# caojiezhang/CiaoSR

Hardware: AMD Instinct MI355X
Metric: HR Mpix/s (RDN-CiaoSR x4, LocalImplicitSR forward_test) (higher is better)
Workload: dtype f32; 1 GPU; C3: RDN-CiaoSR (c64b16) x4, LR 1356x2040 -> 5424x8160 (DIV2K-shaped 2K LR), tiled inference: 117 tiles of 192x192 (overlap 32), random-init weights, fp32; scale=4, tiles=117, parallelism=tile-shard x1

## Files before the change

ciaosr_amd/_lib.py:

```python
import ctypes as C
import os

_HERE = os.path.dirname(os.path.abspath(__file__))
LIB_PATH = os.environ.get('CIAOSR_HIP_LIB') or os.path.join(_HERE, 'csrc', 'libciaosr_hip.so')
MAX_LAYERS = 8

ACT_NONE, ACT_RELU, ACT_PRELU, ACT_GELU, ACT_SIN, ACT_COS = 0, 1, 2, 3, 4, 5


class CiaoSRHipError(RuntimeError):
    pass


class MlpT(C.Structure):
    _fields_ = [('n_layers', C.c_int), ('act', C.c_int), ('in_dim', C.c_int), ('width', C.c_int * MAX_LAYERS),
                ('weight', C.c_void_p * MAX_LAYERS), ('ld', C.c_int * MAX_LAYERS),
                ('bias', C.c_void_p * MAX_LAYERS), ('frag', C.c_void_p * MAX_LAYERS),
                ('frag16', C.c_void_p * MAX_LAYERS), ('frag16_lo', C.c_void_p * MAX_LAYERS)]


class HeadWeightsT(C.Structure):
    _fields_ = [('channels', C.c_int), ('nonlocal_channels', C.c_int), ('nonlocal_max_scale', C.c_int), ('local_size', C.c_int),
                ('no_unfold', C.c_int),
                ('softmax_scale', C.c_float), ('q', MlpT), ('k', MlpT), ('v', MlpT), ('k_out_wino', C.c_void_p), ('k_out_wino4', C.c_void_p),
# ... 6 lines not shown


class CsAttnWeightsT(C.Structure):
    _fields_ = [('channels', C.c_int), ('scale', C.c_int),
                ('w_match1', C.c_void_p), ('b_match1', C.c_void_p), ('slope_match1', C.c_float),
                ('w_match2', C.c_void_p), ('b_match2', C.c_void_p), ('slope_match2', C.c_float),
                ('w_assembly', C.c_void_p), ('b_assembly', C.c_void_p), ('slope_assembly', C.c_float),
                ('w_down', C.c_void_p), ('b_down', C.c_void_p), ('w_down_masked', C.c_void_p),
                ('escape_nan', C.c_float), ('softmax_scale', C.c_float)]


class OptionsT(C.Structure):
    _fields_ = [('head_route', C.c_int), ('csa_composed_min', C.c_int), ('dense_min_tiles', C.c_int),
                ('scatter_small_max', C.c_int), ('kv_rows', C.c_int), ('decode_rows', C.c_int), ('bf16_single', C.c_int),
                ('dense_direct', C.c_int), ('csa_scores_gemm', C.c_int), ('csa_attn_tile128', C.c_int), ('query_grid_w', C.c_int), ('f16_pairs', C.c_int),
                ('csa_attn_v16', C.c_int), ('edsr_resident', C.c_int), ('swin_h16', C.c_int), ('csa_block_mb', C.c_int)]


HEAD_STAGED, HEAD_NO_LOGIT_TABLE, HEAD_TABLE_GEMM, HEAD_WIDE_WG, HEAD_TABLE_WINO2, HEAD_NO_CHAIN, HEAD_NO_DECODE_CHAIN = 1, 2, 4, 8, 16, 32, 64


class ConvT(C.Structure):
    _fields_ = [('weight', C.c_void_p), ('bias', C.c_void_p), ('cin', C.c_int), ('cout', C.c_int), ('ksize', C.c_int),
                ('frag16', C.c_void_p), ('frag16_lo', C.c_void_p), ('frag', C.c_void_p), ('frag_wino', C.c_void_p),
                ('frag_wino4', C.c_void_p)]


class RdnWeightsT(C.Structure):
    _fields_ = [('mid_channels', C.c_int), ('growth', C.c_int), ('num_blocks', C.c_int), ('num_layers', C.c_int),
                ('sfe1', ConvT), ('sfe2', ConvT), ('gff0', ConvT), ('gff1', ConvT),
                ('dense', C.POINTER(ConvT)), ('lff', C.POINTER(ConvT)),
# ... 29 lines not shown
    'ciaosr_sizeof': (_S, [C.c_char_p]),
    'ciaosr_prof_enable': (_I, [_I]),
    'ciaosr_prof_filter': (_I, [C.c_char_p]),
    'ciaosr_prof_reset': (_I, []),
    'ciaosr_prof_collect': (_I, []),
    'ciaosr_prof_get': (_I, [C.c_char_p, C.POINTER(C.c_double), C.POINTER(C.c_long)]),
    'ciaosr_prof_names': (_I, [C.c_char_p, _I]),
    'ciaosr_nchw_to_hwc_f32': (_I, [_P, _P, _I, _I, _I, _I, _P]),
    'ciaosr_hwc_to_nchw_f32': (_I, [_P, _I, _P, _I, _I, _I, _P]),
    'ciaosr_gemm_f32': (_I, [_P, _I, _P, _I, _I, _P, _I, _P, _I, _I, _I, _F, _I, _F, _P]),
    'ciaosr_patch_rows_f32': (_I, [_P, _I, _I, _I, _I, _I, _I, _I, _I, _I, _P, _I, _I, _F, _P]),
    'ciaosr_cs_attn_workspace_bytes': (_S, [_I, _I, _I]),
    'ciaosr_cs_attn_workspace_bytes_scale': (_S, [_I, _I, _I, _I]),
    'ciaosr_cs_attn_workspace_bytes_opt': (_S, [_I, _I, _I, _I, _O]),
    'ciaosr_cs_attn_block_rows': (_I, [_I, _I, _I, _I, _I, _O]),
    'ciaosr_cs_attn_f32': (_I, [_P, _I, _I, _I, C.POINTER(CsAttnWeightsT), _P, _I, _O, _P, _S, _P]),
    'ciaosr_cs_attn_bf16': (_I, [_P, _I, _I, _I, C.POINTER(CsAttnWeightsT), _P, _I, _O, _P, _S, _P]),
    'ciaosr_make_coord_cell_f32': (_I, [_P, _P, _I, _I, _P]),
    'ciaosr_make_coord_cell_window_f32': (_I, [_P, _P, _I, _I, _I, _I, _I, _I, C.POINTER(_I), _P]),
    'ciaosr_fragment_floats': (_S, [_I, _I]),
    'ciaosr_head_decode_rows': (_I, [_I, _I]),
    'ciaosr_pack_fragments_f32': (_I, [_P, _I, _I, _I, _P, _P]),
    'ciaosr_cs_attn_f16': (_I, [_P, _I, _I, _I, C.POINTER(CsAttnWeightsT), _P, _I, _O, _P, _S, _P]),
    'ciaosr_fragment_bf16_bytes': (_S, [_I, _I]),
    'ciaosr_fragment_f16_bytes': (_S, [_I, _I]),
    'ciaosr_pack_fragments_f16': (_I, [_P, _I, _I, _I, _P, _P]),
    'ciaosr_pack_fragments_bf16': (_I, [_P, _I, _I, _I, _P, _P]),
    'ciaosr_pack_fragments_bf16_lo': (_I, [_P, _I, _I, _I, _P, _P]),
    'ciaosr_pack_fragments_f16_lo': (_I, [_P, _I, _I, _I, _P, _P]),
    'ciaosr_pack_fragments_bf16_pair': (_I, [_P, _I, _I, _I, _P, _P, _P]),
# ... 161 lines not shown
```

ciaosr_amd/csrc/common.h:

```cpp
#pragma once
#include <hip/hip_runtime.h>
#include <atomic>
#include <cstdint>
#include <cstdio>
#include <mutex>

#include "../../include/ciaosr_hip.h"

namespace ciaosr {

constexpr int kWave = 64;

static inline int ceil_div(long a, long b) { return (int)((a + b - 1) / b); }

static inline bool aligned16(const void* p) { return (reinterpret_cast<uintptr_t>(p) & 15u) == 0; }

struct ProfScope {
    int slot;
    hipStream_t stream;
    hipEvent_t ev0, ev1;
    ProfScope(const char* name, hipStream_t s);
    ~ProfScope();
};

// ... 19 lines not shown

__device__ __forceinline__ void wave_lds_sync() {
    __builtin_amdgcn_fence(__ATOMIC_RELEASE, "wavefront");
    __builtin_amdgcn_wave_barrier();
    __builtin_amdgcn_fence(__ATOMIC_ACQUIRE, "wavefront");
}

int launch_status(const char* what);

static inline bool options_ok(const ciaosr_options_t* o) {
    if (!o) return true;
    return o->query_grid_w >= 0 && (o->csa_attn_tile128 == 0 || o->csa_attn_tile128 == 1) && (o->head_route & ~127) == 0 && (o->kv_rows == 0 || o->kv_rows == 32 || o->kv_rows == 64) &&
           (o->decode_rows == 0 || o->decode_rows == 32 || o->decode_rows == 64) && (o->bf16_single == 0 || o->bf16_single == 1) &&
           (o->dense_direct >= 0 && o->dense_direct <= 2) && (o->csa_scores_gemm == 0 || o->csa_scores_gemm == 1) &&
           o->f16_pairs >= 0 && o->f16_pairs <= 3 && (o->csa_attn_v16 == 0 || o->csa_attn_v16 == 1) && o->csa_block_mb >= 0 &&
           (o->swin_h16 == 0 || o->swin_h16 == 1) && (o->edsr_resident == 0 || o->edsr_resident == 1);
}

}

#define CIAOSR_BIG_LDS(kernel, bytes)                                                              \
    do {                                                                                           \
        static ::ciaosr::LdsAttrOnce once_;                                                        \
        if (!::ciaosr::allow_big_lds(once_, kernel, bytes)) return CIAOSR_ERR_LAUNCH;              \
    } while (0)

#define CIAOSR_CHECK_ARG(cond)                                                         \
    do {                                                                               \
        if (!(cond)) {                                                                 \
            std::fprintf(stderr, "[ciaosr_hip] bad argument: %s (%s:%d)\n", #cond,     \
                         __FILE__, __LINE__);                                          \
// ... 4 lines not shown
```

ciaosr_amd/csrc/csattn.hip:

```cpp
#include "ops.h"

namespace ciaosr {

struct CsaPlan {
    int H, W, C, sc, Hp, Wp, HWp, Hl, Wl, L, Lld, Lld8, Ch;
    int band_rows, up, down, s_rows;
    size_t n_V, n_S, n_Y;
    bool banded() const { return band_rows < Hp; }
};

static CsaPlan csa_plan(int H, int W, int C, int sc) {
    CsaPlan p;
    p.H = H; p.W = W; p.C = C; p.sc = sc; p.Ch = (int)round_up(C / 2, 4);
    p.Hp = (int)round_up((size_t)H, sc); p.Wp = (int)round_up((size_t)W, sc);
    p.HWp = p.Hp * p.Wp; p.Hl = p.Hp / sc; p.Wl = p.Wp / sc; p.L = p.Hl * p.Wl;
    p.Lld = (int)round_up(p.L, 4); p.Lld8 = (int)round_up(p.L, 8);
    p.band_rows = p.s_rows = p.Hp; p.up = p.down = 0;
    p.n_V = (size_t)p.L * 9 * sc * sc * C; p.n_S = (size_t)p.HWp * p.Lld; p.n_Y = (size_t)sc * sc * p.HWp * C;
    return p;
}

static bool csa_composed(const CsaPlan& p, const ciaosr_options_t* opt) {
    const int composed_min = opt && opt->csa_composed_min ? opt->csa_composed_min : 4096;
    return p.sc == 2 && composed_min > 0 && p.HWp >= composed_min;
// ... 63 lines not shown
    b.Er = p.banded() ? take((size_t)(p.Wp + p.Hp) * p.Lld) : nullptr;
    return b;
}
static size_t csa_carve_bytes(const CsaPlan& p, bool p16) {
    size_t n = 0;
    csa_carve(p, p16, [&](size_t floats) { n += floats; return (float*)nullptr; });
    return n * sizeof(float) + 24 * 256;
}

enum CsaScores { kScoresBox, kScoresGemm, kScores16 };
enum CsaTail { kTailUncomposed, kTail16C, kTailFour, kTail16 };
struct CsaRoute {
    CsaScores scores; CsaTail tail;
    bool tile128;
    bool fused_softmax;
};

static CsaRoute csa_route(const CsaPlan& p, Prec prec, const ciaosr_options_t* opt, const ciaosr_csattn_weights_t* w) {
    CsaRoute r = {kScoresGemm, kTailUncomposed, opt && opt->csa_attn_tile128, false};
    if (prec == kF32 && !(opt && opt->csa_scores_gemm) && csa_scores_box_ok(p.Ch, p.Ch, p.Ch)) r.scores = kScoresBox;
    if (!(csa_composed(p, opt) && w->w_down_masked)) return r;
    if (prec != kF32 && (9 * p.Ch) % 8 == 0 && (p.Lld & 3) == 0 && qk16_fits(p) && vpt_fits(p)) {
        r.scores = kScores16; r.tail = kTail16;
        r.fused_softmax = softmax16_fits(p, h16_ops(prec)) && w->softmax_scale > 0.f;
    } else if (csa_wants_four(p, prec, opt, p.s_rows)) {
        r.tail = kTailFour;
    } else {
        r.tail = kTail16C;
    }
    return r;
}
static bool csa_attn_big(const CsaPlan& p, const CsaRoute& r, int M) {
    return !r.tile128 && gemm_big_softmax_f32_ok(p.Lld, 25 * p.C, M, 16 * p.C, p.L, true) &&
           ((size_t)(M - 1) * p.Lld + p.L) * sizeof(float) < 0xFFFFFF00ull;
}

// ... 54 lines not shown
    int patch_down(const float* src, int Hs, int Ws, int stride, int pad, int OH, int OW, float* dst) const {
        return patch_rows(src, C, Hs, Ws, C, 3, stride, pad, OH, OW, dst, 9 * C, 0, 0.f, s, "csa_patch_down");
    }
    int partial_down() const {
        CSA_RUN(patch_down(E, Hp, Wp, 2, 3, Hl + 3, Wl + 3, PE));
        return gemm_f32(PE, 9 * C, w->w_down_masked, 9 * C, false, Pc, 9 * C, nullptr, (Hl + 3) * (Wl + 3), 9 * C, 9 * C, 1.f, CIAOSR_ACT_NONE, 0.f, s,
                        "csa_down_partial");
    }

    int keep_edge_logits(const CsaBand& b) const {
        if (!banded()) return CIAOSR_OK;
        if (b.first()) CSA_RUN(copy_rows(S, Lld, Wp, Lld, edge_rows(), Lld, s, "csa_edge_rows"));
        return copy_rows(S + (size_t)(b.y0 - b.ya) * Wp * Lld, (long)Wp * Lld, b.y1 - b.y0, Lld, edge_rows() + (size_t)(Wp + b.y0) * Lld, Lld, s,
                         "csa_edge_rows");
    }
    int edges(const float* Vc, int ld, int col0, const float* probs) const {
        auto edge = [&](int pix0, int pix_stride, int col, float* dst, int rows, int n) -> int {
            const float* B = Vc + col0 + col;
            if (probs)
                return gemm_f32_splitk(probs + (size_t)pix0 * Lld, Lld, B, ld, true, dst, n, nullptr, rows, n, L, 1.f, CIAOSR_ACT_NONE, 0.f, splitk(),
                                       n_Y, s, "csa_attn_v_edge");
            const float* A = !banded() ? S : edge_rows() + (size_t)pix0 * Lld;
            return gemm_f32_softmax_a(A, banded() ? Lld : pix_stride * Lld, stats(), pix_stride, B, ld, true, dst, n, rows, n, L, splitk(), n_Y, s,
                                      "csa_attn_v_edge");
        };
        CSA_RUN(edge(0, 1, 0, otop(), Wp, 4 * C));
        CSA_RUN(edge(Wp, Wp, 4 * C, oleft(), Hp, 4 * C));
        return edge(0, 1, 8 * C, otl(), 1, C);
    }
    int finish_16c(const float* probs) const {
        CSA_RUN(edges(Vp, 25 * C, 16 * C, probs));
        return csa_gather_out(O, otop(), oleft(), otl(), w->b_down, H, W, Hp, Wp, C, out, ld_out, 16L * C, 4L * C, 4L * C, s);
    }

    int tail_four(const CsaRoute& r, const CsaBand& b) const {
        CSA_RUN(softmax_stats_rows(S, (long)(b.yb - b.ya) * Wp, L, Lld, stats() + 2 * (size_t)b.ya * Wp, s));
        if (b.first()) {
            CSA_RUN(partial_down());
            CSA_RUN(csa_gather_vedge(Pc, Hl, Wl, C, vedge(), s));
        }
        CSA_RUN(csa_attn_v4_f32(S, Lld, stats(), Pc, partial4(), Hp, Wp, C, r.tile128, b.ya, b.yb - b.ya, b.y0, b.y1, s));
        return keep_edge_logits(b);
    }
    int finish_four() const {
        CSA_RUN(edges(vedge(), 9 * C, 0, nullptr));
        return csa_attn_v4_combine(partial4(), otop(), oleft(), otl(), w->b_down, H, W, Hp, Wp, C, out, ld_out, s);
    }

    int tail_16c(const CsaRoute& r, const CsaBand& b) const {
        const int rows = npix(b, Wp);
        float* st = stats() + 2 * (size_t)b.y0 * Wp;
        float* Ob = O + (size_t)b.y0 * Wp * 16 * C;
        CSA_RUN(softmax_stats_rows(S, rows, L, Lld, st, s));
        if (b.first()) {
            CSA_RUN(partial_down());
            CSA_RUN(csa_gather_vprime(Pc, Hl, Wl, C, Vp, s));
        }
        CSA_RUN(csa_attn_big(*this, r, rows) ? gemm_big_softmax_f32(S, Lld, st, 1, Vp, 25 * C, Ob, 16 * C, rows, 16 * C, L, s, "csa_attn_v")
                                             : gemm_f32_softmax_a(S, Lld, st, 1, Vp, 25 * C, true, Ob, 16 * C, rows, 16 * C, L, nullptr, 0, s, "csa_attn_v"));
        return keep_edge_logits(b);
    }

    int tail_16(Prec prec, const CsaBand& b) const {
        const H16Ops& h = h16_ops(prec); const bool f16 = prec == kF16;
        if (b.first()) {
            CSA_RUN(partial_down());
            CSA_RUN(csa_gather_vprime_t_h16(Pc, Hl, Wl, C, vpT(), Lld8, f16, s));
        }
        CSA_RUN(h.gemm_nt(P16, Lld8, vpT(), Lld8, O + (size_t)b.y0 * Wp * 16 * C, 16 * C, false, npix(b, Wp), 16 * C, Lld8, 1.f, s,
                          f16 ? "csa_attn_v_f16" : "csa_attn_v_bf16", HWp));
        if (!banded()) return CIAOSR_OK;
        if (b.first()) CSA_RUN(h.rows_to_f32(P16, Lld8, 0, 1, Wp, Lld, edge_rows(), Lld, s));
        return h.rows_to_f32(P16, Lld8, 0, Wp, b.y1 - b.y0, Lld, edge_rows() + (size_t)(Wp + b.y0) * Lld, Lld, s);
    }
    int finish_16(Prec prec) const {
        const H16Ops& h = h16_ops(prec);
        CSA_RUN(csa_gather_vprime(Pc, Hl, Wl, C, Vp, s));
        if (!banded()) {
            CSA_RUN(h.rows_to_f32(P16, Lld8, 0, 1, Wp, Lld, edge_rows(), Lld, s));
            CSA_RUN(h.rows_to_f32(P16, Lld8, 0, Wp, Hp, Lld, edge_rows() + (size_t)Wp * Lld, Lld, s));
        }
        return finish_16c(edge_rows());
    }

    int tail_uncomposed(const CsaBand& b) const {
        const int kv = 9 * sc * sc * C, rows = npix(b, Wp);
        CSA_RUN(softmax_rows(S, rows, L, Lld, s));
        if (b.first()) CSA_RUN(patch_rows(E, C, Hp, Wp, C, 3 * sc, sc, sc, Hl, Wl, V, kv, 0, 0.f, s, "csa_patch_v"));
        return gemm_f32(S, Lld, V, kv, true, O + (size_t)b.y0 * Wp * kv, kv, nullptr, rows, kv, L, 1.f, CIAOSR_ACT_NONE, 0.f, s, "csa_attn_v", HWp);
    }
    int finish_uncomposed() const {
        const int kv = 9 * sc * sc * C;
        CSA_RUN(sc == 2 ? fold(O, kv, Hp, Wp, C, Y, s) : fold_s(O, kv, Hp, Wp, C, sc, Y, s));
        CSA_RUN(patch_down(Y, sc * Hp, sc * Wp, sc, 1, H, W, Yp));
        if (gemm_small_ok(H * W, C, 9 * C, 9 * C, 9 * C) && H * W <= 4096)
            return gemm_small_f32(Yp, 9 * C, w->w_down, 9 * C, w->b_down, out, ld_out, nullptr, 0, nullptr, 0, H * W, C, 9 * C, CIAOSR_ACT_NONE, 0.f,
                                  1.0f / 6.0f, s, "csa_down");
// ... 14 lines not shown
extern "C" size_t ciaosr_cs_attn_workspace_bytes_opt(int H, int W, int C, int scale, const ciaosr_options_t* opt) {
    size_t n = 0;
    for (const Prec prec : {kF32, kF16}) {
        CsaPlan p = csa_plan(H, W, C, csa_scale(scale));
        csa_plan_bands(p, prec, opt);
        const size_t m = csa_carve_bytes(p, !p.banded() || prec != kF32);
        n = m > n ? m : n;
    }
    return n;
}
extern "C" int ciaosr_cs_attn_block_rows(int H, int W, int C, int scale, int precision, const ciaosr_options_t* opt) {
    if (H < 1 || W < 1 || C < 1 || scale < 2 || scale > 4 || precision < 0 || precision > 2 || !options_ok(opt)) return 0;
    CsaPlan p = csa_plan(H, W, C, scale);
    csa_plan_bands(p, (Prec)precision, opt);
    return p.band_rows;
}

static int cs_attn(const float* feat_hwc, int ld_feat, int H, int W, const ciaosr_csattn_weights_t* w, float* out, int ld_out,
                   const ciaosr_options_t* opt, void* workspace, size_t workspace_bytes, void* stream, Prec prec) {
    CIAOSR_CHECK_ARG(feat_hwc && w && out && workspace && H >= 2 && W >= 2);
    CIAOSR_CHECK_ARG(options_ok(opt));
    const int C = w->channels, sc = w->scale ? w->scale : 2;
    CIAOSR_CHECK_ARG(C >= 4 && (C & 3) == 0 && ld_feat >= C && (ld_feat & 3) == 0 && (ld_out & 3) == 0);
    CIAOSR_CHECK_ARG(sc >= 2 && sc <= 4 && H >= sc && W >= sc);
    CsaPlan p = csa_plan(H, W, C, sc);
    csa_plan_bands(p, prec, opt);
    const CsaRoute r = csa_route(p, prec, opt, w);
    if (r.tail != kTailFour) p.up = p.down = 0;
    if (workspace_bytes < (p.banded() ? ciaosr_cs_attn_workspace_bytes_opt(H, W, C, sc, opt) : ciaosr_cs_attn_workspace_bytes_scale(H, W, C, sc)))
        return CIAOSR_ERR_WORKSPACE;
    Arena ar(workspace, workspace_bytes);
    const CsaCall c = {csa_carve(p, !p.banded() || prec != kF32, [&](size_t floats) { return ar.take<float>(floats); }), w, out, ld_out,
                       (hipStream_t)stream};
    if (!ar.ok) return CIAOSR_ERR_WORKSPACE;
    CSA_RUN(c.embed(feat_hwc, ld_feat));
    CSA_RUN(c.scores_operands(r, prec));
    for (int y0 = 0; y0 < p.Hp; y0 += p.band_rows) {
        const CsaBand b = c.band(y0);
        CSA_RUN(c.scores(r, prec, b));
        CSA_RUN(r.tail == kTailFour ? c.tail_four(r, b) : r.tail == kTail16C ? c.tail_16c(r, b) : r.tail == kTail16 ? c.tail_16(prec, b)
                                                                                                                   : c.tail_uncomposed(b));
    }
    if (r.tail == kTailFour) return c.finish_four();
    if (r.tail == kTail16C) return c.finish_16c(nullptr);
    if (r.tail == kTail16) return c.finish_16(prec);
    return c.finish_uncomposed();
}

extern "C" int ciaosr_cs_attn_f32(const float* feat_hwc, int ld_feat, int H, int W, const ciaosr_csattn_weights_t* w, float* out, int ld_out,
                                  const ciaosr_options_t* opt, void* workspace, size_t workspace_bytes, void* stream) {
    return cs_attn(feat_hwc, ld_feat, H, W, w, out, ld_out, opt, workspace, workspace_bytes, stream, kF32);
}
extern "C" int ciaosr_cs_attn_bf16(const float* feat_hwc, int ld_feat, int H, int W, const ciaosr_csattn_weights_t* w, float* out, int ld_out,
                                   const ciaosr_options_t* opt, void* workspace, size_t workspace_bytes, void* stream) {
    return cs_attn(feat_hwc, ld_feat, H, W, w, out, ld_out, opt, workspace, workspace_bytes, stream, kBF16);
}
extern "C" int ciaosr_cs_attn_f16(const float* feat_hwc, int ld_feat, int H, int W, const ciaosr_csattn_weights_t* w, float* out, int ld_out,
                                  const ciaosr_options_t* opt, void* workspace, size_t workspace_bytes, void* stream) {
    return cs_attn(feat_hwc, ld_feat, H, W, w, out, ld_out, opt, workspace, workspace_bytes, stream, kF16);
}
// ... 1 lines not shown
```

ciaosr_amd/csrc/gemm_f32.hip:

```cpp
#include <type_traits>

#include "common.h"

namespace ciaosr {

typedef float f32x16 __attribute__((ext_vector_type(16)));

#ifndef CIAOSR_GEMM32_TNK
#define CIAOSR_GEMM32_TNK 24
#endif
#ifndef CIAOSR_GEMM32_BK
#define CIAOSR_GEMM32_BK 16
#endif
constexpr int BM = 128, BN = 128, BK = CIAOSR_GEMM32_BK;
constexpr int F4R = BK / 4;
constexpr int NSA = BM * F4R / 256;
constexpr int NSB = BK * (BN / 4) / 256;
constexpr int LDS_A = BK + 4;
constexpr int LDS_BKN = BN + 4;
constexpr int A_TILE = BM * LDS_A;
constexpr int B_TILE = (BN * LDS_A > BK * LDS_BKN) ? BN * LDS_A : BK * LDS_BKN;

struct GemmP {
    const float* A;
// ... 18 lines not shown
__device__ __forceinline__ float4 buf_ld4(__amdgpu_buffer_rsrc_t rsrc, unsigned byte_off) {
    const i32x4 v = __builtin_amdgcn_raw_buffer_load_b128(rsrc, (int)byte_off, 0, 0);
    return make_float4(__int_as_float(v.x), __int_as_float(v.y), __int_as_float(v.z), __int_as_float(v.w));
}
__device__ __forceinline__ float4 buf_ld4s(__amdgpu_buffer_rsrc_t rsrc, unsigned byte_off, unsigned s_off) {
    const i32x4 v = __builtin_amdgcn_raw_buffer_load_b128(rsrc, (int)byte_off, (int)s_off, 0);
    return make_float4(__int_as_float(v.x), __int_as_float(v.y), __int_as_float(v.z), __int_as_float(v.w));
}
__device__ __forceinline__ float4 mask4(float4 v, int first, int limit) {
    if (first + 1 >= limit) v.y = 0.f;
    if (first + 2 >= limit) v.z = 0.f;
    if (first + 3 >= limit) v.w = 0.f;
    return v;
}

template <bool B_KN, bool MULTI, bool SM = false>
__global__ __launch_bounds__(256, 2) void gemm_f32_kernel(GemmP p) {
    extern __shared__ __attribute__((aligned(16))) float smem[];
    float* As = smem;
    float* Bs = smem + 2 * A_TILE;

    const int bid = blockIdx.x;
    const int q8 = p.n_wg >> 3, r8 = p.n_wg & 7;
    const int xcd = bid & 7, slot = bid >> 3;
    const int lid = (xcd < r8 ? xcd * (q8 + 1) : r8 * (q8 + 1) + (xcd - r8) * q8) + slot;
    const int m0 = (lid / p.groups_n) * BM;
    const int tile0 = (lid % p.groups_n) * p.tn_per_wg;
    const int ntl = min(p.tn_per_wg, p.tiles_n - tile0);

    const int t = threadIdx.x;
    const int lane = t & 63, w = t >> 6;
    const int wm = w >> 1, wn = w & 1;
    const int li = lane & 31, lh = lane >> 5;

    float4 ra[4], rb[4];
    const int nk_total = (p.K + BK - 1) / BK;
    const int kt0 = blockIdx.y * p.kt_per_split;
    const int kt1 = min(nk_total, kt0 + p.kt_per_split);
    const __amdgpu_buffer_rsrc_t rs_a = __builtin_amdgcn_make_buffer_rsrc(const_cast<float*>(p.A), 0, p.a_bytes, 0x00020000);
    const __amdgpu_buffer_rsrc_t rs_b = __builtin_amdgcn_make_buffer_rsrc(const_cast<float*>(p.B), 0, p.b_bytes, 0x00020000);

    unsigned offA[NSA], offB[NSA > NSB ? NSA : NSB];
#pragma unroll
    for (int s = 0; s < NSA; ++s) {
        const int idx = t + 256 * s;
        const int gm = m0 + idx / F4R;
        offA[s] = gm < p.M ? ((unsigned)gm * (unsigned)p.lda + (unsigned)((idx % F4R) * 4)) * 4u : kOobG;
    }
    auto set_cols = [&](int n0) __attribute__((always_inline)) {
        if (!B_KN) {
#pragma unroll
            for (int s = 0; s < NSA; ++s) {
// ... 108 lines not shown

    auto epilogue = [&](int n0) {
#pragma unroll
        for (int ni = 0; ni < 2; ++ni) {
            const int col = n0 + wn * 64 + ni * 32 + li;
            if (col >= p.N) continue;
            const float bv = p.bias ? p.bias[col] : 0.f;
#pragma unroll
            for (int mi = 0; mi < 2; ++mi) {
#pragma unroll
                for (int r = 0; r < 16; ++r) {
                    const int row = m0 + wm * 64 + mi * 32 + (r & 3) + 8 * (r >> 2) + 4 * lh;
                    if (row >= p.M) continue;
                    if constexpr (!MULTI) {
                        if (p.splitk > 1) {
                            p.partial[((size_t)blockIdx.y * p.M + row) * p.N + col] = acc[mi][ni][r];
                            continue;
                        }
                    }
                    float v = (acc[mi][ni][r] + bv) * p.alpha;
                    if constexpr (!MULTI) {
                        if (p.act == CIAOSR_ACT_RELU) v = fmaxf(v, 0.f);
                        else if (p.act == CIAOSR_ACT_PRELU) v = v > 0.f ? v : v * p.slope;
                        else if (p.act == CIAOSR_ACT_SIN) v = sinf(v);
                        else if (p.act == CIAOSR_ACT_COS) v = cosf(v);
                    }
                    p.C[(size_t)row * p.ldc + col] = v;
                }
            }
        }
    };
// ... 45 lines not shown
        if constexpr (MULTI) {
            if (c_kt + 1 == kt1) {
                epilogue(c_tile * BN);
#pragma unroll
                for (int mi = 0; mi < 2; ++mi)
#pragma unroll
                    for (int ni = 0; ni < 2; ++ni)
#pragma unroll
                        for (int r = 0; r < 16; ++r) acc[mi][ni][r] = 0.f;
            }
        }
        c_tile = n_tile; c_kt = n_kt;
        __syncthreads();
    }
    if constexpr (!MULTI) epilogue(tile0 * BN);
}

__global__ void gemm_reduce_kernel(GemmP p) {
    const long n = (long)p.M * p.N;
    for (long i = blockIdx.x * (long)blockDim.x + threadIdx.x; i < n; i += (long)gridDim.x * blockDim.x) {
        float v = 0.f;
        for (int s = 0; s < p.splitk; ++s) v += p.partial[(size_t)s * n + i];
        const int row = (int)(i / p.N), col = (int)(i - (long)row * p.N);
        v = (v + (p.bias ? p.bias[col] : 0.f)) * p.alpha;
        if (p.act == CIAOSR_ACT_RELU) v = fmaxf(v, 0.f);
        else if (p.act == CIAOSR_ACT_PRELU) v = v > 0.f ? v : v * p.slope;
        else if (p.act == CIAOSR_ACT_SIN) v = sinf(v);
        else if (p.act == CIAOSR_ACT_COS) v = cosf(v);
        p.C[(size_t)row * p.ldc + col] = v;
    }
// ... 132 lines not shown
    p.n_wg = ceil_div(M, BM) * p.tiles_n;
    const int nk = (K + BK - 1) / BK;
    p.splitk = 1; p.kt_per_split = nk; p.partial = nullptr;
    if (partial) {
        int splits = ceil_div(512, p.n_wg);
        if (splits > nk / 4) splits = nk / 4 > 0 ? nk / 4 : 1;
        if ((size_t)splits * M * N > partial_floats) splits = (int)(partial_floats / ((size_t)M * N));
        if (splits < 1) splits = 1;
        p.kt_per_split = ceil_div(nk, splits);
        p.splitk = ceil_div(nk, p.kt_per_split);
        p.partial = partial;
    }
    return gemm_launch(p, b_kn, stream, tag);
}

}

extern "C" int ciaosr_gemm_f32(const float* A, int lda, const float* B, int ldb, int b_is_kn, float* C,
                               int ldc, const float* bias, int M, int N, int K, float alpha, int act,
                               float slope, void* stream) {
    return ciaosr::gemm_f32(A, lda, B, ldb, b_is_kn != 0, C, ldc, bias, M, N, K, alpha, act, slope,
                            (hipStream_t)stream, nullptr, 0);
}
```

ciaosr_amd/csrc/ops.h:

```cpp
#pragma once
#include "common.h"

namespace ciaosr {

constexpr int MAXJ = 9;

struct HeadRowsP {
    const float* coord;
    const float* cell;
    long q0;
    int nq, chunk, H, W, local_size, J;
    const float* Tk;
    const float* Tv;
    const float* tailK;
    const float* tailV;
    int ld_tail_k, ld_tail_v;
    int wk0, wv0, relu_k, relu_v;
    float* Hk;
    float* Hv;
    int* q_idx;
    int* k_idx;
};

struct LocalAttnP {
// ... 14 lines not shown
    const float* b;
    const float* x_lr;
    const float* coord;
    long q0;
    int nq, H, W;
    float* rgb;
};

int gemm_f32(const float* A, int lda, const float* B, int ldb, bool b_kn, float* C, int ldc, const float* bias,
             int M, int N, int K, float alpha, int act, float slope, hipStream_t stream, const char* tag, int plan_rows = 0);
int gemm_f32_splitk(const float* A, int lda, const float* B, int ldb, bool b_kn, float* C, int ldc, const float* bias,
                    int M, int N, int K, float alpha, int act, float slope, float* partial, size_t partial_floats,
                    hipStream_t stream, const char* tag);
int gemm_f32_softmax_a(const float* A, int lda, const float* a_stats2, int a_stats_stride, const float* B, int ldb, bool b_kn, float* C, int ldc,
                       int M, int N, int K, float* partial, size_t partial_floats, hipStream_t stream, const char* tag);
bool gemm_big_softmax_f32_ok(int lda, int ldb, int M, int N, int K, bool b_kn);
int gemm_big_softmax_f32(const float* A, int lda, const float* a_stats2, int a_stats_stride, const float* B, int ldb, float* C, int ldc,
                         int M, int N, int K, hipStream_t stream, const char* tag);
bool gemm_small_ok(int M, int N, int K, int lda, int ldw);
int gemm_small_f32(const float* A, int lda, const float* W, int ldw, const float* bias, float* C, int ldc, float* C2, int ldc2,
                   const float* res, int ldres, int M, int N, int K, int act, float slope, float alpha, hipStream_t s, const char* tag);
int dense_wino_tiles(int H, int W);
int dense_layer_wino_f32(float* X, int ldx, int H, int W, int l, const float* frag_wino, const float* bias, int n_img, hipStream_t s);
int dense_wino4_tiles(int H, int W);
int dense_layer_wino4_f32(float* X, int ldx, int H, int W, int l, const float* frag_wino4, const float* bias, int n_img, hipStream_t s);
int wino_table_f32(const float* Pi, int H, int W, const float* frag_wino, int n_blk, float* out, int ldg, hipStream_t s);
int wino4_table_f32(const float* Pi, int H, int W, const float* frag_wino4, int n_blk, float* out, int ldg, hipStream_t s);
bool csa_scores_box_ok(int Ch, int ldm, int ldr);
int csa_key_norms(const float* R, int ldr, int Hl, int Wl, int Ch, float alpha, float floor_, float* nrm, hipStream_t s);
int csa_scores_box_f32(const float* M, int ldm, int Hp, int Wp, const float* R, int ldr, int Hl, int Wl, int Ch, const float* nrm, float* S,
// ... 214 lines not shown
```

ciaosr_amd/csrc/runtime.hip:

```cpp
#include <cstring>
#include "common.h"

#include <mutex>
#include <string>
#include <vector>

namespace ciaosr {

namespace {
struct Pending {
    int slot;
    hipEvent_t a, b;
};
std::mutex g_mu;
bool g_enabled = false;
std::vector<std::string> g_names;
std::vector<double> g_total_ms;
std::vector<long> g_count;
std::vector<Pending> g_pending;
std::vector<hipEvent_t> g_pool;
std::string g_filter;

hipEvent_t get_event() {
    if (!g_pool.empty()) {
// ... 32 lines not shown
}

int launch_status(const char* what) {
    hipError_t e = hipGetLastError();
    if (e != hipSuccess) {
        std::fprintf(stderr, "[ciaosr_hip] launch of %s failed: %s\n", what, hipGetErrorString(e));
        return CIAOSR_ERR_LAUNCH;
    }
    return CIAOSR_OK;
}

}

using namespace ciaosr;

extern "C" int ciaosr_version(void) { return 320; }

extern "C" size_t ciaosr_sizeof(const char* type_name) {
    if (!type_name) return 0;
    const struct { const char* n; size_t s; } tab[] = {
        {"ciaosr_options_t", sizeof(ciaosr_options_t)},
        {"ciaosr_csattn_weights_t", sizeof(ciaosr_csattn_weights_t)},
        {"ciaosr_mlp_t", sizeof(ciaosr_mlp_t)},
        {"ciaosr_head_weights_t", sizeof(ciaosr_head_weights_t)},
        {"ciaosr_head_scene_t", sizeof(ciaosr_head_scene_t)},
        {"ciaosr_conv_t", sizeof(ciaosr_conv_t)},
        {"ciaosr_rdn_weights_t", sizeof(ciaosr_rdn_weights_t)},
        {"ciaosr_edsr_weights_t", sizeof(ciaosr_edsr_weights_t)},
        {"ciaosr_swin_block_t", sizeof(ciaosr_swin_block_t)},
        {"ciaosr_swinir_weights_t", sizeof(ciaosr_swinir_weights_t)},
    };
// ... 75 lines not shown
```

ciaosr_amd/hip_ops.py:

```python
import ctypes as C
from collections import namedtuple

import torch

from . import _lib
from ._lib import CiaoSRHipError

_workspaces = {}


def require_gpu(*tensors, allow_row_stride=False):
    dev = None
    for t in tensors:
        if t is None:
            continue
        if t.is_cuda:
            if dev is None:
                dev = torch.cuda.current_device()
            if t.device.index != dev:
                raise CiaoSRHipError(f'tensor on cuda:{t.device.index} but the current device is cuda:{dev}: '
                                     f'run the call under torch.cuda.device({t.device.index})')
        if not t.is_cuda:
            raise CiaoSRHipError('the LocalImplicitSR path runs on the MI355X only: got a CPU tensor '
                                 '(no CPU fallback; move the model and inputs to cuda)')
# ... 323 lines not shown
        raise ValueError(f'unknown precision {precision!r}: one of {PRECISIONS} (or an alias: {sorted(_ALIASES)})')
    m = MODES[name]
    pairs = m.f16_pairs if f16_pairs is None else int(f16_pairs)
    single = m.bf16_single if bf16_single is None else int(bf16_single)
    if pairs not in (0, 1, 2, 3) or single not in (0, 1):
        raise ValueError(f'f16_pairs must be 0..3 and bf16_single 0 or 1, got {pairs} / {single}')
    if m.precision == 'fp32':
        return m
    if m.precision == 'bf16':
        return MODES['bf16x3' if pairs == 2 else 'bf16-single' if single else 'bf16']
    return MODES[('f16', 'f16-pairs', 'f16x3', 'f16x3-fast')[pairs]]


class Options:
    _C_FIELDS = ('head_route', 'csa_composed_min', 'dense_min_tiles', 'scatter_small_max', 'kv_rows', 'decode_rows', 'bf16_single', 'dense_direct', 'csa_scores_gemm', 'csa_attn_tile128', 'query_grid_w', 'f16_pairs',
                 'csa_attn_v16', 'edsr_resident', 'swin_h16', 'csa_block_mb')
    _MODE_FIELDS = ('precision', 'f16_pairs', 'bf16_single')
    __slots__ = ('mode', 'precision') + _C_FIELDS + ('_c',)

    def __init__(self, precision='fp32', f16_pairs=None, bf16_single=None, **kw):
        mode = resolve_mode(precision, f16_pairs, bf16_single)
        object.__setattr__(self, 'mode', mode)
        for f in self._MODE_FIELDS:
            object.__setattr__(self, f, getattr(mode, f))
        for f in self._C_FIELDS:
            if f not in self._MODE_FIELDS:
                object.__setattr__(self, f, int(kw.pop(f, 0)))
        if kw:
            raise TypeError(f'unknown option(s): {sorted(kw)}')
        st = None
        if any(getattr(self, f) for f in self._C_FIELDS):
# ... 130 lines not shown
```

include/ciaosr_hip.h:

```cpp
#ifndef CIAOSR_HIP_H
#define CIAOSR_HIP_H

#include <stddef.h>

#ifdef __cplusplus
extern "C" {
#endif

#define CIAOSR_OK 0
#define CIAOSR_ERR_BAD_ARG (-1)
#define CIAOSR_ERR_LAUNCH (-2)
#define CIAOSR_ERR_UNSUPPORTED (-3)
#define CIAOSR_ERR_WORKSPACE (-4)

#define CIAOSR_ACT_NONE 0
#define CIAOSR_ACT_RELU 1
#define CIAOSR_ACT_PRELU 2
#define CIAOSR_ACT_GELU 3
#define CIAOSR_ACT_SIN 4
#define CIAOSR_ACT_COS 5

#define CIAOSR_MAX_LAYERS 8

int ciaosr_version(void);
// ... 16 lines not shown
#define CIAOSR_HEAD_NO_DECODE_CHAIN 64
typedef struct ciaosr_options {
    int head_route;
    int csa_composed_min;
    int dense_min_tiles;
    int scatter_small_max;
    int kv_rows;
    int decode_rows;
    int bf16_single;
    int dense_direct;
    int csa_scores_gemm;
    int csa_attn_tile128;
    int query_grid_w;
    int f16_pairs;
    int csa_attn_v16;
    int edsr_resident;
    int swin_h16;
    int csa_block_mb;
} ciaosr_options_t;

int ciaosr_nchw_to_hwc_f32(const float* src, float* dst, int C, int H, int W, int ld_dst, void* stream);
int ciaosr_hwc_to_nchw_f32(const float* src, int ld_src, float* dst, int C, int H, int W, void* stream);

int ciaosr_gemm_f32(const float* A, int lda, const float* B, int ldb, int b_is_kn, float* C, int ldc,
                    const float* bias, int M, int N, int K, float alpha, int act, float slope,
                    void* stream);

int ciaosr_patch_rows_f32(const float* src_hwc, int ld_src, int Hs, int Ws, int Cs, int ksize, int stride,
                          int pad, int OH, int OW, float* out, int ld_out, int l2_normalize,
                          float norm_floor, void* stream);
// ... 9 lines not shown
    float slope_match2;
    const float* w_assembly;
    const float* b_assembly;
    float slope_assembly;
    const float* w_down;
    const float* b_down;
    const float* w_down_masked;
    float escape_nan;
    float softmax_scale;
} ciaosr_csattn_weights_t;

size_t ciaosr_cs_attn_workspace_bytes(int H, int W, int C);
size_t ciaosr_cs_attn_workspace_bytes_scale(int H, int W, int C, int scale);
size_t ciaosr_cs_attn_workspace_bytes_opt(int H, int W, int C, int scale, const ciaosr_options_t* opt );
int ciaosr_cs_attn_block_rows(int H, int W, int C, int scale, int precision, const ciaosr_options_t* opt );
int ciaosr_cs_attn_f32(const float* feat_hwc, int ld_feat, int H, int W, const ciaosr_csattn_weights_t* w,
                       float* out, int ld_out, const ciaosr_options_t* opt , void* workspace,
                       size_t workspace_bytes, void* stream);
int ciaosr_cs_attn_bf16(const float* feat_hwc, int ld_feat, int H, int W, const ciaosr_csattn_weights_t* w,
                        float* out, int ld_out, const ciaosr_options_t* opt , void* workspace,
                        size_t workspace_bytes, void* stream);
int ciaosr_cs_attn_f16(const float* feat_hwc, int ld_feat, int H, int W, const ciaosr_csattn_weights_t* w,
                       float* out, int ld_out, const ciaosr_options_t* opt , void* workspace,
                       size_t workspace_bytes, void* stream);

typedef struct ciaosr_mlp {
    int n_layers;
    int act;
    int in_dim;
    int width[CIAOSR_MAX_LAYERS];
// ... 348 lines not shown
```

Baseline: 12.20 Mpix/s.

## Group cross-scale attention edge GEMMs into one split-K launch with in-kernel reduction

Adds a grouped f32 GEMM kernel that runs up to three independent GEMM problems in a single launch, using split-K with atomic arrival counters so the last workgroup per tile does the partial-sum reduction in-kernel. The f32 cross-scale attention path (C=64, composed tail, no softmax probs) now computes its top, left and top-left edge products through this grouped launch instead of separate per-edge GEMMs and reduce kernels. This is meant to cut launch overhead and raise occupancy on these small, K-heavy GEMMs. The cost is a memset of the arrival counters, partial-buffer traffic, and extra atomic synchronisation. A new option can turn it off, and a route-code query is exported.

Result: no change. 12.22 Mpix/s (median of 6 runs) (+0.1%).

```diff
diff --git a/ciaosr_amd/_lib.py b/ciaosr_amd/_lib.py
--- a/ciaosr_amd/_lib.py
+++ b/ciaosr_amd/_lib.py
@@ -44,7 +44,7 @@
     _fields_ = [('head_route', C.c_int), ('csa_composed_min', C.c_int), ('dense_min_tiles', C.c_int),
                 ('scatter_small_max', C.c_int), ('kv_rows', C.c_int), ('decode_rows', C.c_int), ('bf16_single', C.c_int),
                 ('dense_direct', C.c_int), ('csa_scores_gemm', C.c_int), ('csa_attn_tile128', C.c_int), ('query_grid_w', C.c_int), ('f16_pairs', C.c_int),
-                ('csa_attn_v16', C.c_int), ('edsr_resident', C.c_int), ('swin_h16', C.c_int), ('csa_block_mb', C.c_int)]
+                ('csa_attn_v16', C.c_int), ('csa_edge_split', C.c_int), ('edsr_resident', C.c_int), ('swin_h16', C.c_int), ('csa_block_mb', C.c_int)]
 
 
 HEAD_STAGED, HEAD_NO_LOGIT_TABLE, HEAD_TABLE_GEMM, HEAD_WIDE_WG, HEAD_TABLE_WINO2, HEAD_NO_CHAIN, HEAD_NO_DECODE_CHAIN = 1, 2, 4, 8, 16, 32, 64
@@ -104,6 +104,7 @@
     'ciaosr_cs_attn_workspace_bytes_scale': (_S, [_I, _I, _I, _I]),
     'ciaosr_cs_attn_workspace_bytes_opt': (_S, [_I, _I, _I, _I, _O]),
     'ciaosr_cs_attn_block_rows': (_I, [_I, _I, _I, _I, _I, _O]),
+    'ciaosr_cs_attn_route_code': (_I, [_I, _I, C.POINTER(CsAttnWeightsT), _I, _O]),
     'ciaosr_cs_attn_f32': (_I, [_P, _I, _I, _I, C.POINTER(CsAttnWeightsT), _P, _I, _O, _P, _S, _P]),
     'ciaosr_cs_attn_bf16': (_I, [_P, _I, _I, _I, C.POINTER(CsAttnWeightsT), _P, _I, _O, _P, _S, _P]),
     'ciaosr_make_coord_cell_f32': (_I, [_P, _P, _I, _I, _P]),
diff --git a/ciaosr_amd/csrc/common.h b/ciaosr_amd/csrc/common.h
--- a/ciaosr_amd/csrc/common.h
+++ b/ciaosr_amd/csrc/common.h
@@ -57,7 +57,8 @@
            (o->decode_rows == 0 || o->decode_rows == 32 || o->decode_rows == 64) && (o->bf16_single == 0 || o->bf16_single == 1) &&
            (o->dense_direct >= 0 && o->dense_direct <= 2) && (o->csa_scores_gemm == 0 || o->csa_scores_gemm == 1) &&
            o->f16_pairs >= 0 && o->f16_pairs <= 3 && (o->csa_attn_v16 == 0 || o->csa_attn_v16 == 1) && o->csa_block_mb >= 0 &&
-           (o->swin_h16 == 0 || o->swin_h16 == 1) && (o->edsr_resident == 0 || o->edsr_resident == 1);
+           (o->swin_h16 == 0 || o->swin_h16 == 1) && (o->edsr_resident == 0 || o->edsr_resident == 1) &&
+           (o->csa_edge_split == 0 || o->csa_edge_split == 1);
 }
 
 }
diff --git a/ciaosr_amd/csrc/csattn.hip b/ciaosr_amd/csrc/csattn.hip
--- a/ciaosr_amd/csrc/csattn.hip
+++ b/ciaosr_amd/csrc/csattn.hip
@@ -101,12 +101,15 @@
     CsaScores scores; CsaTail tail;
     bool tile128;
     bool fused_softmax;
-};
+    bool edge_one;
+};
+constexpr int kCsaEdgeSlices = 24;
 
 static CsaRoute csa_route(const CsaPlan& p, Prec prec, const ciaosr_options_t* opt, const ciaosr_csattn_weights_t* w) {
-    CsaRoute r = {kScoresGemm, kTailUncomposed, opt && opt->csa_attn_tile128, false};
+    CsaRoute r = {kScoresGemm, kTailUncomposed, opt && opt->csa_attn_tile128, false, false};
     if (prec == kF32 && !(opt && opt->csa_scores_gemm) && csa_scores_box_ok(p.Ch, p.Ch, p.Ch)) r.scores = kScoresBox;
     if (!(csa_composed(p, opt) && w->w_down_masked)) return r;
+    r.edge_one = prec == kF32 && p.C == 64 && !(opt && opt->csa_edge_split);
     if (prec != kF32 && (9 * p.Ch) % 8 == 0 && (p.Lld & 3) == 0 && qk16_fits(p) && vpt_fits(p)) {
         r.scores = kScores16; r.tail = kTail16;
         r.fused_softmax = softmax16_fits(p, h16_ops(prec)) && w->softmax_scale > 0.f;
@@ -191,7 +194,17 @@
         return copy_rows(S + (size_t)(b.y0 - b.ya) * Wp * Lld, (long)Wp * Lld, b.y1 - b.y0, Lld, edge_rows() + (size_t)(Wp + b.y0) * Lld, Lld, s,
                          "csa_edge_rows");
     }
-    int edges(const float* Vc, int ld, int col0, const float* probs) const {
+    int edges(const CsaRoute& r, const float* Vc, int ld, int col0, const float* probs) const {
+        if (r.edge_one && !probs) {
+            const float *A1 = !banded() ? S : edge_rows() + (size_t)Wp * Lld, *B = Vc + col0;
+            const int ld0 = Lld, ld1 = banded() ? Lld : Wp * Lld;
+            const GemmProblem eg[3] = {{!banded() ? S : edge_rows(), ld0, stats(), 1, B, ld, otop(), 4 * C, Wp, 4 * C, L},
+                                       {A1, ld1, stats(), Wp, B + 4 * C, ld, oleft(), 4 * C, Hp, 4 * C, L},
+                                       {!banded() ? S : edge_rows(), ld0, stats(), 1, B + 8 * C, ld, otl(), C, 1, C, L}};
+            const size_t words = (size_t)HWp * C;
+            if (gemm_f32_group_ok(eg, 3, true, kCsaEdgeSlices, n_Y, words))
+                return gemm_f32_group(eg, 3, true, kCsaEdgeSlices, splitk(), n_Y, reinterpret_cast<unsigned*>(xp), words, s, "csa_attn_v_edge");
+        }
         auto edge = [&](int pix0, int pix_stride, int col, float* dst, int rows, int n) -> int {
             const float* B = Vc + col0 + col;
             if (probs)
@@ -205,8 +218,8 @@
         CSA_RUN(edge(Wp, Wp, 4 * C, oleft(), Hp, 4 * C));
         return edge(0, 1, 8 * C, otl(), 1, C);
     }
-    int finish_16c(const float* probs) const {
-        CSA_RUN(edges(Vp, 25 * C, 16 * C, probs));
+    int finish_16c(const CsaRoute& r, const float* probs) const {
+        CSA_RUN(edges(r, Vp, 25 * C, 16 * C, probs));
         return csa_gather_out(O, otop(), oleft(), otl(), w->b_down, H, W, Hp, Wp, C, out, ld_out, 16L * C, 4L * C, 4L * C, s);
     }
 
@@ -219,8 +232,8 @@
         CSA_RUN(csa_attn_v4_f32(S, Lld, stats(), Pc, partial4(), Hp, Wp, C, r.tile128, b.ya, b.yb - b.ya, b.y0, b.y1, s));
         return keep_edge_logits(b);
     }
-    int finish_four() const {
-        CSA_RUN(edges(vedge(), 9 * C, 0, nullptr));
+    int finish_four(const CsaRoute& r) const {
+        CSA_RUN(edges(r, vedge(), 9 * C, 0, nullptr));
         return csa_attn_v4_combine(partial4(), otop(), oleft(), otl(), w->b_down, H, W, Hp, Wp, C, out, ld_out, s);
     }
 
@@ -250,14 +263,14 @@
         if (b.first()) CSA_RUN(h.rows_to_f32(P16, Lld8, 0, 1, Wp, Lld, edge_rows(), Lld, s));
         return h.rows_to_f32(P16, Lld8, 0, Wp, b.y1 - b.y0, Lld, edge_rows() + (size_t)(Wp + b.y0) * Lld, Lld, s);
     }
-    int finish_16(Prec prec) const {
+    int finish_16(const CsaRoute& r, Prec prec) const {
         const H16Ops& h = h16_ops(prec);
         CSA_RUN(csa_gather_vprime(Pc, Hl, Wl, C, Vp, s));
         if (!banded()) {
             CSA_RUN(h.rows_to_f32(P16, Lld8, 0, 1, Wp, Lld, edge_rows(), Lld, s));
             CSA_RUN(h.rows_to_f32(P16, Lld8, 0, Wp, Hp, Lld, edge_rows() + (size_t)Wp * Lld, Lld, s));
         }
-        return finish_16c(edge_rows());
+        return finish_16c(r, edge_rows());
     }
 
     int tail_uncomposed(const CsaBand& b) const {
@@ -302,6 +315,16 @@
     CsaPlan p = csa_plan(H, W, C, scale);
     csa_plan_bands(p, (Prec)precision, opt);
     return p.band_rows;
+}
+
+extern "C" int ciaosr_cs_attn_route_code(int H, int W, const ciaosr_csattn_weights_t* w, int precision, const ciaosr_options_t* opt) {
+    CIAOSR_CHECK_ARG(w && H >= 2 && W >= 2 && precision >= kF32 && precision <= kF16 && options_ok(opt));
+    const int C = w->channels, sc = w->scale ? w->scale : 2;
+    CIAOSR_CHECK_ARG(C >= 4 && (C & 3) == 0 && sc >= 2 && sc <= 4 && H >= sc && W >= sc);
+    CsaPlan p = csa_plan(H, W, C, sc);
+    csa_plan_bands(p, (Prec)precision, opt);
+    const CsaRoute r = csa_route(p, (Prec)precision, opt, w);
+    return (int)r.scores | (int)r.tail << 2 | (r.tile128 ? 1 : 0) << 4 | (r.fused_softmax ? 1 : 0) << 5 | (r.edge_one ? 1 : 0) << 6;
 }
 
 static int cs_attn(const float* feat_hwc, int ld_feat, int H, int W, const ciaosr_csattn_weights_t* w, float* out, int ld_out,
@@ -329,9 +352,9 @@
         CSA_RUN(r.tail == kTailFour ? c.tail_four(r, b) : r.tail == kTail16C ? c.tail_16c(r, b) : r.tail == kTail16 ? c.tail_16(prec, b)
                                                                                                                    : c.tail_uncomposed(b));
     }
-    if (r.tail == kTailFour) return c.finish_four();
-    if (r.tail == kTail16C) return c.finish_16c(nullptr);
-    if (r.tail == kTail16) return c.finish_16(prec);
+    if (r.tail == kTailFour) return c.finish_four(r);
+    if (r.tail == kTail16C) return c.finish_16c(r, nullptr);
+    if (r.tail == kTail16) return c.finish_16(r, prec);
     return c.finish_uncomposed();
 }
 
diff --git a/ciaosr_amd/csrc/gemm_f32.hip b/ciaosr_amd/csrc/gemm_f32.hip
--- a/ciaosr_amd/csrc/gemm_f32.hip
+++ b/ciaosr_amd/csrc/gemm_f32.hip
@@ -1,6 +1,6 @@
 #include <type_traits>
 
-#include "common.h"
+#include "ops.h"
 
 namespace ciaosr {
 
@@ -56,16 +56,19 @@
     return v;
 }
 
-template <bool B_KN, bool MULTI, bool SM = false>
-__global__ __launch_bounds__(256, 2) void gemm_f32_kernel(GemmP p) {
+__device__ __forceinline__ int gemm_tile_of(const GemmP& p, int bid) {
+    const int q8 = p.n_wg >> 3, r8 = p.n_wg & 7;
+    const int xcd = bid & 7, slot = bid >> 3;
+    return (xcd < r8 ? xcd * (q8 + 1) : r8 * (q8 + 1) + (xcd - r8) * q8) + slot;
+}
+
+template <bool B_KN, bool MULTI, bool SM>
+__device__ __forceinline__ void gemm_f32_workgroup(const GemmP& p, const int bid, const int ky) {
     extern __shared__ __attribute__((aligned(16))) float smem[];
     float* As = smem;
     float* Bs = smem + 2 * A_TILE;
 
-    const int bid = blockIdx.x;
-    const int q8 = p.n_wg >> 3, r8 = p.n_wg & 7;
-    const int xcd = bid & 7, slot = bid >> 3;
-    const int lid = (xcd < r8 ? xcd * (q8 + 1) : r8 * (q8 + 1) + (xcd - r8) * q8) + slot;
+    const int lid = gemm_tile_of(p, bid);
     const int m0 = (lid / p.groups_n) * BM;
     const int tile0 = (lid % p.groups_n) * p.tn_per_wg;
     const int ntl = min(p.tn_per_wg, p.tiles_n - tile0);
@@ -77,7 +80,7 @@
 
     float4 ra[4], rb[4];
     const int nk_total = (p.K + BK - 1) / BK;
-    const int kt0 = blockIdx.y * p.kt_per_split;
+    const int kt0 = ky * p.kt_per_split;
     const int kt1 = min(nk_total, kt0 + p.kt_per_split);
     const __amdgpu_buffer_rsrc_t rs_a = __builtin_amdgcn_make_buffer_rsrc(const_cast<float*>(p.A), 0, p.a_bytes, 0x00020000);
     const __amdgpu_buffer_rsrc_t rs_b = __builtin_amdgcn_make_buffer_rsrc(const_cast<float*>(p.B), 0, p.b_bytes, 0x00020000);
@@ -216,7 +219,7 @@
                     if (row >= p.M) continue;
                     if constexpr (!MULTI) {
                         if (p.splitk > 1) {
-                            p.partial[((size_t)blockIdx.y * p.M + row) * p.N + col] = acc[mi][ni][r];
+                            p.partial[((size_t)ky * p.M + row) * p.N + col] = acc[mi][ni][r];
                             continue;
                         }
                     }
@@ -292,6 +295,90 @@
         __syncthreads();
     }
     if constexpr (!MULTI) epilogue(tile0 * BN);
+}
+
+template <bool B_KN, bool MULTI, bool SM = false>
+__global__ __launch_bounds__(256, 2) void gemm_f32_kernel(GemmP p) {
+    gemm_f32_workgroup<B_KN, MULTI, SM>(p, blockIdx.x, blockIdx.y);
+}
+
+constexpr int kGemmGroupMax = 3;
+struct GemmGroupP {
+    GemmP g[kGemmGroupMax];
+    int n, wg0[kGemmGroupMax + 1];
+    unsigned* arrivals;
+};
+
+template <bool B_KN, bool SM>
+__global__ __launch_bounds__(256, 2) void gemm_f32_group_kernel(GemmGroupP P) {
+    extern __shared__ __attribute__((aligned(16))) float smem[];
+    int gi = 0;
+#pragma unroll
+    for (int i = 1; i < kGemmGroupMax; ++i)
+        if (i < P.n && (int)blockIdx.x >= P.wg0[i]) gi = i;
+    const GemmP& p = P.g[gi];
+    const int bid = blockIdx.x - P.wg0[gi];
+    gemm_f32_workgroup<B_KN, false, SM>(p, bid, blockIdx.y);
+    if (p.splitk <= 1) return;
+
+    const int t = threadIdx.x;
+    asm volatile("s_waitcnt vmcnt(0)" ::: "memory");
+    __syncthreads();
+    int* const last = reinterpret_cast<int*>(smem);
+    if (t == 0) {
+        __builtin_amdgcn_fence(__ATOMIC_RELEASE, "agent");
+        asm volatile("s_waitcnt vmcnt(0)" ::: "memory");
+        const unsigned ticket = __hip_atomic_fetch_add(P.arrivals + P.wg0[gi] + bid, 1u, __ATOMIC_RELAXED, __HIP_MEMORY_SCOPE_AGENT);
+        const bool is_last = ticket == (unsigned)p.splitk - 1;
+        if (is_last) {
+            __builtin_amdgcn_fence(__ATOMIC_ACQUIRE, "agent");
+            asm volatile("s_waitcnt vmcnt(0)" ::: "memory");
+        }
+        *last = is_last;
+    }
+    __syncthreads();
+    if (!*last) return;
+
+    const int lid = gemm_tile_of(p, bid);
+    const int m0 = (lid / p.groups_n) * BM, n0 = (lid % p.groups_n) * BN;
+    const int rows = min(BM, p.M - m0), cols4 = min(BN, p.N - n0) >> 2;
+    constexpr int NR = BM * BN / 4 / 256;
+    const unsigned slab = (unsigned)p.M * (unsigned)p.N * 4u;
+    const __amdgpu_buffer_rsrc_t rs = __builtin_amdgcn_make_buffer_rsrc(p.partial, 0, (unsigned)p.splitk * slab, 0x00020000);
+    unsigned off[NR];
+    float4 v[NR];
+#pragma unroll
+    for (int j = 0; j < NR; ++j) {
+        const int i = t + 256 * j;
+        const int row = m0 + i / cols4, col = n0 + (i % cols4) * 4;
+        off[j] = i < rows * cols4 ? ((unsigned)row * (unsigned)p.N + (unsigned)col) * 4u : kOobG;
+        v[j] = make_float4(0.f, 0.f, 0.f, 0.f);
+    }
+    auto add = [&](const float4 (&x)[NR]) __attribute__((always_inline)) {
+#pragma unroll
+        for (int j = 0; j < NR; ++j) { v[j].x += x[j].x; v[j].y += x[j].y; v[j].z += x[j].z; v[j].w += x[j].w; }
+    };
+    int s = 0;
+    for (; s + 1 < p.splitk; s += 2) {
+        float4 x0[NR], x1[NR];
+#pragma unroll
+        for (int j = 0; j < NR; ++j) x0[j] = buf_ld4s(rs, off[j], (unsigned)s * slab);
+#pragma unroll
+        for (int j = 0; j < NR; ++j) x1[j] = buf_ld4s(rs, off[j], (unsigned)(s + 1) * slab);
+        add(x0);
+        add(x1);
+    }
+    if (s < p.splitk) {
+        float4 x0[NR];
+#pragma unroll
+        for (int j = 0; j < NR; ++j) x0[j] = buf_ld4s(rs, off[j], (unsigned)s * slab);
+        add(x0);
+    }
+#pragma unroll
+    for (int j = 0; j < NR; ++j) {
+        const int i = t + 256 * j;
+        if (i < rows * cols4) *reinterpret_cast<float4*>(p.C + (size_t)(m0 + i / cols4) * p.ldc + n0 + (i % cols4) * 4) = v[j];
+    }
 }
 
 __global__ void gemm_reduce_kernel(GemmP p) {
@@ -454,6 +541,77 @@
     return gemm_launch(p, b_kn, stream, tag);
 }
 
+static size_t gemm_extent(int rows, int ld, int cols) { return ((size_t)(rows - 1) * ld + cols) * sizeof(float); }
+static int gemm_group_slices(const GemmProblem* g, int n, int slices, size_t partial_floats) {
+    const int nk = (g[0].K + BK - 1) / BK;
+    size_t out = 0;
+    for (int i = 0; i < n; ++i) out += (size_t)g[i].M * g[i].N;
+    int s = slices;
+    if (s > nk / 4) s = nk / 4 > 0 ? nk / 4 : 1;
+    if ((size_t)s * out > partial_floats) s = (int)(partial_floats / out);
+    if ((size_t)s * out * sizeof(float) >= 0xFFFFFF00ull) s = (int)(0xFFFFFF00ull / sizeof(float) / out);
+    return s;
+}
+bool gemm_f32_group_ok(const GemmProblem* g, int n, bool b_kn, int slices, size_t partial_floats, size_t arrival_words) {
+    if (!g || n < 1 || n > kGemmGroupMax || slices < 1) return false;
+    size_t tiles = 0;
+    for (int i = 0; i < n; ++i) {
+        const GemmProblem& q = g[i];
+        if (q.M <= 0 || q.N <= 0 || q.K <= 0 || !q.A || !q.B || !q.C || (q.lda & 3) || (q.ldb & 3) || !aligned16(q.A) || !aligned16(q.B)) return false;
+        if (!q.a_stats2 != !g[0].a_stats2 || (q.a_stats2 && (q.a_stats_stride < 1 || (reinterpret_cast<uintptr_t>(q.a_stats2) & 7u)))) return false;
+        if (gemm_extent(q.M, q.lda, q.K) >= 0xFFFFFF00ull) return false;
+        if ((b_kn ? gemm_extent(q.K, q.ldb, q.N) : gemm_extent(q.N, q.ldb, q.K)) >= 0xFFFFFF00ull) return false;
+        if (q.K != g[0].K || (q.N & 3) || (q.ldc & 3) || !aligned16(q.C)) return false;
+        tiles += (size_t)ceil_div(q.M, BM) * ceil_div(q.N, BN);
+    }
+    return tiles < 0x7FFFFFFF && ((tiles + 3) & ~(size_t)3) <= arrival_words && gemm_group_slices(g, n, slices, partial_floats) >= 1;
+}
+
+int gemm_f32_group(const GemmProblem* g, int n, bool b_kn, int slices, float* partial, size_t partial_floats, unsigned* arrivals,
+                   size_t arrival_words, hipStream_t stream, const char* tag) {
+    CIAOSR_CHECK_ARG(partial && arrivals && aligned16(arrivals) && gemm_f32_group_ok(g, n, b_kn, slices, partial_floats, arrival_words));
+    GemmGroupP P;
+    P.n = n; P.arrivals = arrivals; P.wg0[0] = 0;
+    const int splits = gemm_group_slices(g, n, slices, partial_floats);
+    int splitk = 1;
+    for (int i = 0; i < n; ++i) {
+        const GemmProblem& q = g[i];
+        GemmP& p = P.g[i];
+        p.A = q.A; p.B = q.B; p.C = q.C; p.bias = nullptr;
+        p.M = q.M; p.N = q.N; p.K = q.K; p.lda = q.lda; p.ldb = q.ldb; p.ldc = q.ldc;
+        p.alpha = 1.f; p.slope = 0.f; p.act = CIAOSR_ACT_NONE;
+        p.a_stats = reinterpret_cast<const float2*>(q.a_stats2); p.a_stats_stride = q.a_stats_stride;
+        p.a_bytes = (unsigned)gemm_extent(q.M, q.lda, q.K);
+        p.b_bytes = (unsigned)(b_kn ? gemm_extent(q.K, q.ldb, q.N) : gemm_extent(q.N, q.ldb, q.K));
+        p.tiles_n = ceil_div(q.N, BN); p.tn_per_wg = 1; p.groups_n = p.tiles_n;
+        p.n_wg = ceil_div(q.M, BM) * p.tiles_n;
+        const int nk = (q.K + BK - 1) / BK;
+        p.kt_per_split = ceil_div(nk, splits);
+        p.splitk = splitk = ceil_div(nk, p.kt_per_split);
+        p.partial = partial;
+        partial += (size_t)p.splitk * q.M * q.N;
+        P.wg0[i + 1] = P.wg0[i] + p.n_wg;
+    }
+    for (int i = n; i < kGemmGroupMax; ++i) { P.g[i] = P.g[0]; P.wg0[i + 1] = P.wg0[n]; }
+    const size_t smem = (size_t)(2 * A_TILE + 2 * B_TILE) * sizeof(float);
+    CIAOSR_BIG_LDS((gemm_f32_group_kernel<true, false>), smem);
+    CIAOSR_BIG_LDS((gemm_f32_group_kernel<false, false>), smem);
+    CIAOSR_BIG_LDS((gemm_f32_group_kernel<true, true>), smem);
+    CIAOSR_BIG_LDS((gemm_f32_group_kernel<false, true>), smem);
+    ProfScope prof(tag ? tag : "gemm_f32_group", stream);
+    if (splitk > 1 && hipMemsetAsync(arrivals, 0, ((size_t)P.wg0[n] * sizeof(unsigned) + 15) & ~(size_t)15, stream) != hipSuccess) return CIAOSR_ERR_LAUNCH;
+    const dim3 grid(P.wg0[n], splitk);
+    const bool sm = g[0].a_stats2 != nullptr;
+    if (b_kn) {
+        if (sm) hipLaunchKernelGGL((gemm_f32_group_kernel<true, true>), grid, dim3(256), smem, stream, P);
+        else hipLaunchKernelGGL((gemm_f32_group_kernel<true, false>), grid, dim3(256), smem, stream, P);
+    } else {
+        if (sm) hipLaunchKernelGGL((gemm_f32_group_kernel<false, true>), grid, dim3(256), smem, stream, P);
+        else hipLaunchKernelGGL((gemm_f32_group_kernel<false, false>), grid, dim3(256), smem, stream, P);
+    }
+    return launch_status("gemm_f32_group");
+}
+
 }
 
 extern "C" int ciaosr_gemm_f32(const float* A, int lda, const float* B, int ldb, int b_is_kn, float* C,
diff --git a/ciaosr_amd/csrc/ops.h b/ciaosr_amd/csrc/ops.h
--- a/ciaosr_amd/csrc/ops.h
+++ b/ciaosr_amd/csrc/ops.h
@@ -52,6 +52,13 @@
                     hipStream_t stream, const char* tag);
 int gemm_f32_softmax_a(const float* A, int lda, const float* a_stats2, int a_stats_stride, const float* B, int ldb, bool b_kn, float* C, int ldc,
                        int M, int N, int K, float* partial, size_t partial_floats, hipStream_t stream, const char* tag);
+struct GemmProblem {
+    const float* A; int lda; const float* a_stats2; int a_stats_stride;
+    const float* B; int ldb; float* C; int ldc; int M, N, K;
+};
+bool gemm_f32_group_ok(const GemmProblem* g, int n, bool b_kn, int slices, size_t partial_floats, size_t arrival_words);
+int gemm_f32_group(const GemmProblem* g, int n, bool b_kn, int slices, float* partial, size_t partial_floats, unsigned* arrivals,
+                   size_t arrival_words, hipStream_t stream, const char* tag);
 bool gemm_big_softmax_f32_ok(int lda, int ldb, int M, int N, int K, bool b_kn);
 int gemm_big_softmax_f32(const float* A, int lda, const float* a_stats2, int a_stats_stride, const float* B, int ldb, float* C, int ldc,
                          int M, int N, int K, hipStream_t stream, const char* tag);
diff --git a/ciaosr_amd/csrc/runtime.hip b/ciaosr_amd/csrc/runtime.hip
--- a/ciaosr_amd/csrc/runtime.hip
+++ b/ciaosr_amd/csrc/runtime.hip
@@ -70,7 +70,7 @@
 
 using namespace ciaosr;
 
-extern "C" int ciaosr_version(void) { return 320; }
+extern "C" int ciaosr_version(void) { return 330; }
 
 extern "C" size_t ciaosr_sizeof(const char* type_name) {
     if (!type_name) return 0;
diff --git a/ciaosr_amd/hip_ops.py b/ciaosr_amd/hip_ops.py
--- a/ciaosr_amd/hip_ops.py
+++ b/ciaosr_amd/hip_ops.py
@@ -361,7 +361,7 @@
 
 class Options:
     _C_FIELDS = ('head_route', 'csa_composed_min', 'dense_min_tiles', 'scatter_small_max', 'kv_rows', 'decode_rows', 'bf16_single', 'dense_direct', 'csa_scores_gemm', 'csa_attn_tile128', 'query_grid_w', 'f16_pairs',
-                 'csa_attn_v16', 'edsr_resident', 'swin_h16', 'csa_block_mb')
+                 'csa_attn_v16', 'csa_edge_split', 'edsr_resident', 'swin_h16', 'csa_block_mb')
     _MODE_FIELDS = ('precision', 'f16_pairs', 'bf16_single')
     __slots__ = ('mode', 'precision') + _C_FIELDS + ('_c',)
 
diff --git a/include/ciaosr_hip.h b/include/ciaosr_hip.h
--- a/include/ciaosr_hip.h
+++ b/include/ciaosr_hip.h
@@ -54,6 +54,7 @@
     int query_grid_w;
     int f16_pairs;
     int csa_attn_v16;
+    int csa_edge_split;
     int edsr_resident;
     int swin_h16;
     int csa_block_mb;
@@ -93,6 +94,7 @@
 size_t ciaosr_cs_attn_workspace_bytes_scale(int H, int W, int C, int scale);
 size_t ciaosr_cs_attn_workspace_bytes_opt(int H, int W, int C, int scale, const ciaosr_options_t* opt );
 int ciaosr_cs_attn_block_rows(int H, int W, int C, int scale, int precision, const ciaosr_options_t* opt );
+int ciaosr_cs_attn_route_code(int H, int W, const ciaosr_csattn_weights_t* w, int precision, const ciaosr_options_t* opt );
 int ciaosr_cs_attn_f32(const float* feat_hwc, int ld_feat, int H, int W, const ciaosr_csattn_weights_t* w,
                        float* out, int ld_out, const ciaosr_options_t* opt , void* workspace,
                        size_t workspace_bytes, void* stream);
```
